# jaesung-cs/vulkan_radix_sort

Measured on AMD Instinct MI355X. Metric: GItems/s at N=2^25 (keys & key+value); achieved HBM GB/s vs peak, higher is better.
Workload: dtype u32

## Files before the change

### vulkan_radix_sort_amd/csrc/vrdx_kernels.hip

```cpp
#include <hip/hip_runtime.h>
#include <stdint.h>

#include <type_traits>

#include "vrdx_kernels.h"
#include "vrdx_layout.h"

namespace vrdx {



#ifdef VRDX_TRACE
#define VRDX_STAMP(slot)                                      \
  do {                                                        \
    if (a.trace != nullptr && tid == 0) stamps[slot] = wall_clock64(); \
  } while (0)
#else
#define VRDX_STAMP(slot) \
  do {                   \
  } while (0)
#endif


typedef uint32_t u32x4 __attribute__((ext_vector_type(4)));
typedef uint32_t u32x2 __attribute__((ext_vector_type(2)));
typedef u32x4 u32x4_a4 __attribute__((aligned(4)));

__device__ __forceinline__ uint32_t LoadStatus(const uint32_t* p) {
  return __hip_atomic_load(p, __ATOMIC_RELAXED, __HIP_MEMORY_SCOPE_AGENT);
}
__device__ __forceinline__ void StoreStatus(uint32_t* p, uint32_t v) {
  __hip_atomic_store(p, v, __ATOMIC_RELAXED, __HIP_MEMORY_SCOPE_AGENT);
}

__device__ __forceinline__ void AddToBlock(uint32_t* p, uint32_t count) {
  (void)__hip_atomic_fetch_add(p, count | (1u << VRDX_BLOCK_COUNT_SHIFT), __ATOMIC_RELAXED, __HIP_MEMORY_SCOPE_AGENT);
}

__device__ __forceinline__ uint32_t ElementCount(uint32_t maxCount, const uint32_t* countPtr) {
  if (countPtr == nullptr) return maxCount;
  const uint32_t c = *countPtr;
  return c < maxCount ? c : maxCount;
}

__device__ __forceinline__ uint64_t MatchDigit(uint32_t digit) {
  uint64_t mask = ~0ull;
#pragma unroll
  for (int b = 0; b < 8; ++b) {
    const bool bit = (digit >> b) & 1u;
    const uint64_t ballot = __ballot(bit);
    mask &= bit ? ballot : ~ballot;
  }
  return mask;
}

__device__ __forceinline__ uint32_t LanesBelow(uint64_t mask) {
  return __builtin_amdgcn_mbcnt_hi((uint32_t)(mask >> 32),
                                   __builtin_amdgcn_mbcnt_lo((uint32_t)mask, 0u));
}

__device__ __forceinline__ void LdsBarrier() {
  __builtin_amdgcn_fence(__ATOMIC_RELEASE, "workgroup", "local");
  __builtin_amdgcn_s_barrier();
  __builtin_amdgcn_fence(__ATOMIC_ACQUIRE, "workgroup", "local");
}

template <int KPT, bool NT = false, bool DYN = false>
__device__ __forceinline__ void LoadStriped(const uint32_t* base, uint32_t first, uint32_t n, bool full,
                                            uint32_t pad, uint32_t (&out)[KPT], uint32_t slots = KPT) {
  const char* const bytes = reinterpret_cast<const char*>(base);
  const uint32_t offset = first * 4u;
  auto word = [&](int i) {
    const uint32_t* const p = reinterpret_cast<const uint32_t*>(bytes + ((uint64_t)offset + (uint64_t)(i * 256)));
    return NT ? __builtin_nontemporal_load(p) : *p;
  };
  if (full) {
#pragma unroll
    for (int i = 0; i < KPT; ++i) {
      if (DYN && i % 4 == 0 && (uint32_t)i >= slots) break;
      out[i] = word(i);
    }
  } else {
#pragma unroll
    for (int i = 0; i < KPT; ++i) {
      if (DYN && i % 4 == 0 && (uint32_t)i >= slots) break;
      out[i] = first + i * 64 < n ? word(i) : pad;
    }
  }
}

__device__ __forceinline__ bool StreamingLoads(bool keyValue, uint32_t n) {
  return keyValue && n > kStreamingLoadsAbove && n <= kStreamingLoadsUpTo;
}

template <int KPT, bool DYN = false>
__device__ __forceinline__ void LoadTile(const uint32_t* base, uint32_t first, uint32_t n, bool full, uint32_t pad,
                                         uint32_t (&out)[KPT], bool streaming, uint32_t slots = KPT) {
  if (streaming) {
    asm volatile("; non-temporal tile loads" ::: "memory");
    LoadStriped<KPT, true, DYN>(base, first, n, full, pad, out, slots);
    asm volatile("" ::: "memory");
  } else {
    LoadStriped<KPT, false, DYN>(base, first, n, full, pad, out, slots);
  }
}

template <int KPT, bool DYN = false>
__device__ __forceinline__ void StoreStriped(uint32_t* base, uint32_t first, uint32_t n, bool full,
                                             const uint32_t (&in)[KPT], uint32_t slots = KPT) {
  char* const bytes = reinterpret_cast<char*>(base);
  const uint32_t offset = first * 4u;
#pragma unroll
  for (int i = 0; i < KPT; ++i) {
    if (DYN && i % 4 == 0 && (uint32_t)i >= slots) break;
    if (full || first + i * 64 < n)
      *reinterpret_cast<uint32_t*>(bytes + ((uint64_t)offset + (uint64_t)(i * 256))) = in[i];
  }
}

struct PassPlan {
  bool skip;
  bool copy;
  bool fromScratch;
  uint32_t digit;
};


template <int THREADS>
struct PassCounts {
  uint32_t v[(VRDX_PASSES * VRDX_RADIX) / THREADS];
};

template <int THREADS>
__device__ __forceinline__ PassCounts<THREADS> LoadPassCounts(const uint32_t* histogramTable, int tid) {
  PassCounts<THREADS> c;
#pragma unroll
  for (int k = 0; k < (int)(VRDX_PASSES * VRDX_RADIX) / THREADS; ++k) c.v[k] = histogramTable[tid + k * THREADS];
  return c;
}

template <int THREADS>
__device__ __forceinline__ void PublishPassVotes(const PassCounts<THREADS>& c, uint32_t n, uint32_t hybridCap, int tid,
                                                 uint32_t* flags) {
#pragma unroll
  for (int k = 0; k < (int)(VRDX_PASSES * VRDX_RADIX) / THREADS; ++k) {
    const int group = (tid + k * THREADS) >> 6;
    const uint64_t any = __ballot(c.v[k] == n);
    const uint64_t over = __ballot(c.v[k] > hybridCap);
    if ((tid & 63) == 0) {
      flags[group] = any != 0ull ? 1u : 0u;
      flags[16 + group] = over != 0ull ? 1u : 0u;
    }
  }
}

__device__ __forceinline__ uint32_t TrivialPasses(const uint32_t* flags) {
  uint32_t trivial = 0;
#pragma unroll
  for (uint32_t q = 0; q < VRDX_PASSES; ++q)
    if ((flags[4 * q] | flags[4 * q + 1] | flags[4 * q + 2] | flags[4 * q + 3]) != 0) trivial |= 1u << q;
  return trivial;
}

__device__ __forceinline__ int HybridByte(const uint32_t* flags, uint32_t hybridCap) {
  if (hybridCap == 0) return -1;
  const uint32_t ranked = ~TrivialPasses(flags) & 15u;
  if (ranked == 0) return -1;
  const int top = 31 - __clz((int)ranked);
  const bool fits = (flags[16 + 4 * top] | flags[17 + 4 * top] | flags[18 + 4 * top] | flags[19 + 4 * top]) == 0;
  return fits ? top : -1;
}

__device__ __forceinline__ PassPlan ReadPassPlan(const uint32_t* flags, uint32_t pass, uint32_t hybridCap) {
  PassPlan plan;
  const int hybridByte = HybridByte(flags, hybridCap);
  if (hybridByte >= 0) {
    plan.skip = pass != 0;
    plan.copy = false;
    plan.fromScratch = false;
    plan.digit = (uint32_t)hybridByte;
    return plan;
  }
  const uint32_t trivial = TrivialPasses(flags);
  const uint32_t ranked = VRDX_PASSES - (uint32_t)__popc(trivial);
  const uint32_t copier = (ranked & 1u) ? (uint32_t)(__ffs(trivial) - 1) : VRDX_PASSES;
  const uint32_t changes = (~trivial & 15u) | (copier < VRDX_PASSES ? 1u << copier : 0u);
  plan.skip = ((changes >> pass) & 1u) == 0;
  plan.copy = !plan.skip && ((trivial >> pass) & 1u) != 0;
  plan.fromScratch = (__popc(changes & ((1u << pass) - 1u)) & 1) != 0;
  plan.digit = pass;
  return plan;
}

__device__ __forceinline__ uint32_t WaveInclusiveScan(uint32_t v) {
  int x = (int)v;
  x += __builtin_amdgcn_update_dpp(0, x, 0x111, 0xf, 0xf, true);
  x += __builtin_amdgcn_update_dpp(0, x, 0x112, 0xf, 0xf, true);
  x += __builtin_amdgcn_update_dpp(0, x, 0x114, 0xf, 0xf, true);
  x += __builtin_amdgcn_update_dpp(0, x, 0x118, 0xf, 0xf, true);
  x += __builtin_amdgcn_update_dpp(0, x, 0x142, 0xa, 0xf, false);
  x += __builtin_amdgcn_update_dpp(0, x, 0x143, 0xc, 0xf, false);
  return (uint32_t)x;
}

__device__ __forceinline__ uint32_t BlockExclusiveScan256(uint32_t v, uint32_t* scratch4, int tid) {
  const int lane = tid & 63;
  const int wave = tid >> 6;
  const uint32_t x = WaveInclusiveScan(v);
  if (wave < 4 && lane == 63) scratch4[wave] = x;
  LdsBarrier();
  uint32_t add = 0;
  if (wave < 4) {
#pragma unroll
    for (int w = 0; w < 3; ++w)
      if (w < wave) add += scratch4[w];
  }
  return x - v + add;
}

constexpr uint32_t kHistGroupVecs = kHistGroupKeys / 4;
static_assert(kHistGroupVecs == kHistThreads * 4, "four loads per lane and group");

template <bool NT>
__device__ __forceinline__ void HistFetch(const u32x4_a4* keys4, uint32_t group, uint32_t tid, uint32_t nvec,
                                          u32x4 (&k)[4]) {
#pragma unroll
  for (uint32_t u = 0; u < 4; ++u) {
    uint32_t i = group * kHistGroupVecs + u * kHistThreads + tid;
    i = i < nvec ? i : (nvec != 0 ? nvec - 1 : 0u);
    k[u] = NT ? __builtin_nontemporal_load(keys4 + i) : keys4[i];
  }
}

template <uint32_t COPIES>
__global__ __launch_bounds__(kHistThreads) void histogram_kernel(const uint32_t* __restrict__ keys,
                                                                  uint32_t maxCount,
                                                                  const uint32_t* countPtr,
                                                                  uint32_t* __restrict__ globalHistogram,
                                                                  uint32_t* __restrict__ tickets,
                                                                  u32x4* __restrict__ statusClear,
// ... 1768 lines not shown
        LdsBarrier();
      }
      auto finish = [&](uint32_t done) {
        if (done == nvec / tileVecs && tid < (n & 3u)) {
          const uint32_t one[1] = {keys[(nvec << 2) + tid]};
          count(formTag, kOne, one);
        }
        if constexpr (FORM != TABLES) {
          flush(done, window);
          window = window == top ? top + kTopHalf : top;
        }
      };
      if (two) {
        for (; tile < tiles; tile += step) {
          tally(formTag, tile, 0, a4, nvec);
          fetch(streaming, tile + step, 0, nvec, a4);
          tally(formTag, tile, 4, b4, nvec);
          fetch(streaming, tile + step, 4, nvec, b4);
          finish(tile);
        }
      } else {
        for (; tile < tiles; tile += 2 * step) {
          tally(formTag, tile, 0, a4, nvec);
          fetch(streaming, tile + 2 * step, 0, nvec, a4);
          finish(tile);
          tally(formTag, tile + step, 0, b4, nvec);
          fetch(streaming, tile + 3 * step, 0, nvec, b4);
          if (tile + step < tiles) finish(tile + step);
        }
      }
    };
    if (form == TOP)
      loop(std::integral_constant<uint32_t, TOP>{});
    else if (form == PREFIXED)
      loop(std::integral_constant<uint32_t, PREFIXED>{});
    else
      loop(std::integral_constant<uint32_t, TABLES>{});
  };
  if (n > kHistStreamingLoadsAbove) {
    asm volatile("; non-temporal key loads" ::: "memory");
    sweep(std::true_type{});
  } else {
    sweep(std::false_type{});
  }
  if (form == PREFIXED && likeRef != 0u) atomicAdd(&byte3[(ref >> 24) * C3 + (tid & (C3 - 1))], likeRef);
  __syncthreads();

  if (tid < 3 * VRDX_RADIX) {
    uint32_t sum = 0;
#pragma unroll
    for (uint32_t c = 0; c < COPIES; ++c) sum += bins[tid * COPIES + ((c + tid) & (COPIES - 1))];
    if (sum != 0) atomicAdd(&a.histogramTable[tid], sum);
  } else {
    const uint32_t v = tid - 3 * VRDX_RADIX;
    uint32_t sum = 0;
    if (form == TOP) {
#pragma unroll
      for (uint32_t q = 0; q < PER_BYTE; ++q) sum += bucketSize[v * PER_BYTE + q];
    } else if (form == PREFIXED) {
#pragma unroll
      for (uint32_t c = 0; c < C3; ++c) sum += byte3[v * C3 + ((c + tid) & (C3 - 1))];
    } else {
#pragma unroll
      for (uint32_t c = 0; c < COPIES; ++c) sum += top[v * COPIES + ((c + tid) & (COPIES - 1))];
    }
    if (sum != 0) atomicAdd(&a.histogramTable[tid], sum);
  }
  if (form == PREFIXED) {
    for (uint32_t d = tid; d < D; d += kHistThreads) {
      const uint32_t mine = bucketSize[d];
      if (mine != 0) atomicAdd(&a.bucketCount[d], mine);
    }
  }
  const uint32_t above = shift + BITS;
  const bool broken = form == PREFIXED ? (differs >> (above & 31u)) != 0u : (mode == kMsdModeIdentical && differs != 0u);
  if (__ballot(broken) != 0ull && lane == 0) atomicOr(a.overflowWord, kMsdDeclinePrefix);
}

template <uint32_t BITS>
__global__ __launch_bounds__(1024) void spine_msd_kernel(MsdArgs a) {
  constexpr uint32_t D = 1u << BITS, ROW = D / 2;
  constexpr uint32_t WORDS = 16, CHUNKS = 64, MAXROWS = kMsdMaxTiles / CHUNKS;
  __shared__ uint32_t sumLo[WORDS][CHUNKS], sumHi[WORDS][CHUNKS], total[2 * WORDS], below[16];
  const uint32_t tid = threadIdx.x;
  const uint32_t j = tid & (WORDS - 1), c = tid / WORDS;
  const uint32_t w = blockIdx.x * WORDS + j;
  const uint32_t rows = (a.tiles + CHUNKS - 1) / CHUNKS;
  const uint32_t r0 = c * rows;
  uint32_t* const column = a.tileCounts + w;
  const uint32_t decided = *a.overflowWord;

  {
    u32x4* const clear = reinterpret_cast<u32x4*>(a.statusClear);
    for (uint32_t i = blockIdx.x * 1024u + tid; i < a.statusVecs; i += gridDim.x * 1024u) clear[i] = u32x4{0u, 0u, 0u, 0u};
  }
  const uint32_t firstBucket = blockIdx.x * 2u * WORDS;
  uint32_t underTop = tid < 256u && tid < (firstBucket >> (BITS - 8u)) ? a.histogramTable[3u * VRDX_RADIX + tid] : 0u;
  uint32_t underSizes = 0;
#pragma unroll
  for (uint32_t d = tid; d < D; d += 1024u)
    if (d < firstBucket) underSizes += a.bucketCount[d];

  uint32_t v[MAXROWS];
#pragma unroll
  for (uint32_t k = 0; k < MAXROWS; ++k) v[k] = (k < rows && r0 + k < a.tiles) ? column[(size_t)(r0 + k) * ROW] : 0u;
  if ((decided & kMsdDeclineMask) != 0u || ((decided >> kMsdModeShift) & kMsdModeMask) != kMsdModePlan) return;
  const bool topWindow = ((decided >> kMsdShiftShift) & kMsdShiftMask) == 32u - BITS;
  uint32_t under = topWindow ? underTop : underSizes;
  uint32_t lo = 0, hi = 0;
#pragma unroll
  for (uint32_t k = 0; k < MAXROWS; ++k) {
    lo += v[k] & 0xFFFFu;
    hi += v[k] >> 16;
  }
  sumLo[j][c] = lo;
  sumHi[j][c] = hi;
  under = WaveInclusiveScan(under);
  if ((tid & 63u) == 63u) below[tid >> 6] = under;
  __syncthreads();
  {
    const uint32_t word = tid >> 6, chunk = tid & 63u;
    const uint32_t x = sumLo[word][chunk], y = sumHi[word][chunk];
    const uint32_t ix = WaveInclusiveScan(x), iy = WaveInclusiveScan(y);
    sumLo[word][chunk] = ix - x;
    sumHi[word][chunk] = iy - y;
    if (chunk == 63u) {
      total[2 * word] = ix;
      total[2 * word + 1] = iy;
    }
  }
  __syncthreads();
  lo = sumLo[j][c];
  hi = sumHi[j][c];
#pragma unroll
  for (uint32_t k = 0; k < MAXROWS; ++k) {
    if (k < rows && r0 + k < a.tiles) column[(size_t)(r0 + k) * ROW] = (lo & 0xFFFFu) | (hi << 16);
    lo += v[k] & 0xFFFFu;
    hi += v[k] >> 16;
  }
  if (tid < 64u) {
    const uint32_t mine = tid < 2 * WORDS ? total[tid] : 0u;
    const uint32_t inclusive = WaveInclusiveScan(mine);
    if (tid < 2 * WORDS) {
      uint32_t base = inclusive - mine;
#pragma unroll
      for (uint32_t q = 0; q < 16; ++q) base += below[q];
      a.bucketBase[firstBucket + tid] = base;
      if (topWindow) a.bucketCount[firstBucket + tid] = mine;
      if (mine > a.cap) atomicOr(a.overflowWord, kMsdDeclineBucket);
    }
  }
}

template <uint32_t BITS, bool KV>
__device__ __forceinline__ void ScatterMsdBody(const MsdArgs a) {
  constexpr int THREADS = 1024, KPT = 32, WAVES = THREADS / 64;
  constexpr uint32_t TILE = kMsdTileKeys, D = 1u << BITS, ROW = D / 2u;
  static_assert(THREADS * KPT == TILE && ROW <= (uint32_t)THREADS && WAVES * ROW <= TILE, "geometry");
  extern __shared__ __attribute__((aligned(16))) uint32_t smem[];
  uint32_t* const sorted = smem;
  uint32_t* const counters = smem;
  uint32_t* const tileOffset = smem + TILE;
  uint32_t* const scanScratch = tileOffset + D;

  const int tid = threadIdx.x;
  const int lane = tid & 63;
  const int wave = tid >> 6;
  const uint32_t n = ElementCount(a.maxCount, a.countPtr);
  const uint32_t perXcd = gridDim.x / 8u;
  const uint32_t tile = (blockIdx.x % 8u) * perXcd + blockIdx.x / 8u;
  const uint32_t slots = a.tileKeys / (uint32_t)THREADS;
  const uint32_t frame = a.tileKeys;
  const uint32_t tileStart = tile * frame;
  const uint32_t decided = *a.overflowWord;
  if ((decided & kMsdDeclineMask) != 0u) {
    if (blockIdx.x == 0 && tid == 0 && a.declinedPlans != nullptr) atomicAdd(a.declinedPlans, 1u);
    return;
  }
  const uint32_t SHIFT = (decided >> kMsdShiftShift) & kMsdShiftMask;
  if (((decided >> kMsdModeShift) & kMsdModeMask) == kMsdModeIdentical) {
    if (blockIdx.x == 0 && tid == 0) *a.planWord = kMsdVerdictSorted;
    return;
  }
  const uint32_t valid = tile < a.tiles && tileStart < n ? ((n - tileStart) < frame ? (n - tileStart) : frame) : 0u;
  const uint32_t tileEnd = tileStart + valid;
  const uint32_t loadBase = tileStart + wave * (slots * 64) + lane;
  uint32_t key[KPT];
  LoadStriped<KPT, true, true>(a.keysCaller, loadBase, tileEnd, valid == frame, 0xFFFFFFFFu, key, slots);
  uint32_t prefixWord = 0, base0 = 0, base1 = 0;
  if ((uint32_t)tid < ROW && valid != 0) {
    prefixWord = a.tileCounts[(size_t)tile * ROW + tid];
    base0 = a.bucketBase[2 * tid];
    base1 = a.bucketBase[2 * tid + 1];
  }
  if (blockIdx.x == 0 && tid == 0) *a.planWord = kMsdVerdictRuns | (SHIFT << kMsdShiftShift);
  if (valid == 0) return;

  uint32_t* const myRow = counters + wave * ROW;
#pragma unroll
  for (uint32_t i = 0; i < ROW / 256u; ++i) reinterpret_cast<u32x4*>(myRow)[lane + 64 * i] = u32x4{0u, 0u, 0u, 0u};
  uint32_t rank[KPT / 2];
  RankPacked16<KPT, true>(key, SHIFT, BITS, myRow, lane, rank, slots);
  ForgetDerivedValues<KPT>(key);
  LdsBarrier();

  uint32_t column[WAVES];
  const uint32_t totals = (uint32_t)tid < ROW ? ColumnRead<ROW, WAVES>(counters, tid, column) : 0u;
  const uint32_t count0 = totals & 0xFFFFu, count1 = totals >> 16;
  const uint32_t local0 = BlockExclusiveScanAll<THREADS>(count0 + count1, scanScratch, tid);
  const uint32_t local1 = local0 + count0;
  if ((uint32_t)tid < ROW) {
    ColumnBasesFrom<ROW, WAVES>(counters, tid, local0 | (local1 << 16), column);
    tileOffset[2 * tid] = base0 + (prefixWord & 0xFFFFu) - local0;
    tileOffset[2 * tid + 1] = base1 + (prefixWord >> 16) - local1;
  }
  LdsBarrier();
  PositionsPacked16<KPT, TILE, true>(key, SHIFT, BITS, myRow, rank, slots);
  LdsBarrier();
#pragma unroll
  for (int i = 0; i < KPT; ++i) {
    if (i % 4 == 0 && (uint32_t)i >= slots) break;
    sorted[(rank[i / 2] >> (16 * (i % 2))) & 0xFFFFu] = key[i];
  }
  LdsBarrier();
  uint32_t val[KV ? KPT : 1];
  if constexpr (KV)
    LoadStriped<KPT, true, true>(a.valuesCaller, loadBase, tileEnd, valid == frame, 0u, val, slots);

  constexpr int QUADS = KPT / 4;
  constexpr int B = 4;
  uint32_t quadDigits[KV ? QUADS : 1];
  uint32_t boundaryQuad[2] = {~0u, ~0u};
  uint32_t boundaryDigits[2][2] = {{0, 0}, {0, 0}};
  if ((uint32_t)tid < ROW) {
    if (count0 != 0 && (local0 & 3u) != 0 && local0 < valid) boundaryQuad[0] = local0 & ~3u;
    if (count1 != 0 && (local1 & 3u) != 0 && local1 < valid) boundaryQuad[1] = local1 & ~3u;
  }
  if (tid == 0 && (valid & 3u) != 0) boundaryQuad[0] = valid & ~3u;
  auto scatterQuads = [&](uint32_t* out, bool keysPhase) {
#pragma unroll
    for (int j0 = 0; j0 < QUADS; j0 += B) {
      if (4u * (uint32_t)j0 * THREADS >= valid) break;
      u32x4 w4[B];
      uint32_t o[B];
      bool whole[B];
#pragma unroll
      for (int b = 0; b < B; ++b) w4[b] = *reinterpret_cast<const u32x4*>(&sorted[4u * (tid + (j0 + b) * THREADS)]);
#pragma unroll
      for (int b = 0; b < B; ++b) {
        const int j = j0 + b;
        const uint32_t p = StagingSlot<TILE>(4u * (tid + j * THREADS));
        uint32_t d0, d3;
        if (keysPhase) {
          d0 = __builtin_amdgcn_ubfe(w4[b][0], SHIFT, BITS);
          d3 = __builtin_amdgcn_ubfe(w4[b][3], SHIFT, BITS);
          if constexpr (KV) quadDigits[j] = d0 | (d3 << 16);
        } else {
          d0 = quadDigits[KV ? j : 0] & 0xFFFFu;
          d3 = quadDigits[KV ? j : 0] >> 16;
        }
        whole[b] = p + 3 < valid && d0 == d3;
        o[b] = tileOffset[d0] + p;
        asm volatile("" : "+v"(o[b]));
      }
#pragma unroll
      for (int b = 0; b < B; ++b)
        if (whole[b]) StoreQuad(out, o[b], w4[b]);
    }
#pragma unroll
    for (int s = 0; s < 2; ++s) {
      if (boundaryQuad[s] == ~0u) continue;
      const u32x4 q = *reinterpret_cast<const u32x4*>(&sorted[StagingSlot<TILE>(boundaryQuad[s])]);
      if (keysPhase) {
        boundaryDigits[s][0] = __builtin_amdgcn_ubfe(q[0], SHIFT, BITS) | (__builtin_amdgcn_ubfe(q[1], SHIFT, BITS) << 16);
        boundaryDigits[s][1] = __builtin_amdgcn_ubfe(q[2], SHIFT, BITS) | (__builtin_amdgcn_ubfe(q[3], SHIFT, BITS) << 16);
      }
#pragma unroll
      for (int c = 0; c < 4; ++c) {
        const uint32_t d = (boundaryDigits[s][c / 2] >> (16 * (c % 2))) & 0xFFFFu;
        if (boundaryQuad[s] + c < valid) StoreWord(out, tileOffset[d] + boundaryQuad[s] + c, q[c]);
      }
    }
  };
  scatterQuads(a.keysScratch, true);
  if constexpr (KV) {
    LdsBarrier();
#pragma unroll
    for (int i = 0; i < KPT; ++i) {
      if (i % 4 == 0 && (uint32_t)i >= slots) break;
      sorted[(rank[i / 2] >> (16 * (i % 2))) & 0xFFFFu] = val[i];
    }
    LdsBarrier();
    scatterQuads(a.valuesScratch, false);
  }
}

template <uint32_t BITS>
__device__ __forceinline__ void ScatterMsdPairBody(const MsdArgs a) {
  constexpr int THREADS = 1024, KPT = 32, WAVES = THREADS / 64;
  constexpr uint32_t TILE = kMsdTileKeys, D = 1u << BITS, ROW = D / 2u;
  static_assert(2 * WAVES * ROW <= TILE, "both sub-tiles' counter rows inside the staging buffer");
  extern __shared__ __attribute__((aligned(16))) uint32_t smem[];
  uint32_t* const sorted = smem;
  uint32_t* const counters = smem;
  uint32_t* const tileOffset = smem + TILE;
  uint32_t* const scanScratch = tileOffset + D;

  const int tid = threadIdx.x;
  const int lane = tid & 63;
  const int wave = tid >> 6;
  const uint32_t n = ElementCount(a.maxCount, a.countPtr);
  const uint32_t pairs = (a.tiles + 1u) / 2u;
  const uint32_t perXcd = (pairs + 7u) / 8u;
  const uint32_t pair = (blockIdx.x % 8u) * perXcd + blockIdx.x / 8u;
  const uint32_t slots = a.tileKeys / (uint32_t)THREADS;
  const uint32_t frame = a.tileKeys;
  const uint32_t decided = *a.overflowWord;
  if ((decided & kMsdDeclineMask) != 0u) {
    if (blockIdx.x == 0 && tid == 0 && a.declinedPlans != nullptr) atomicAdd(a.declinedPlans, 1u);
    return;
  }
  const uint32_t SHIFT = (decided >> kMsdShiftShift) & kMsdShiftMask;
  if (((decided >> kMsdModeShift) & kMsdModeMask) == kMsdModeIdentical) {
    if (blockIdx.x == 0 && tid == 0) *a.planWord = kMsdVerdictSorted;
    return;
  }
  const uint32_t tileA = 2u * pair;
  const uint32_t startA = tileA * frame, startB = startA + frame;
  const bool exists = blockIdx.x < 8u * perXcd && pair < pairs && startA < n;
  const uint32_t left = exists ? n - startA : 0u;
  const uint32_t validA = left < frame ? left : frame;
  const uint32_t validB = left > frame ? (left - frame < frame ? left - frame : frame) : 0u;
  const uint32_t valid = validA + validB;
  const uint32_t baseA = startA + wave * (slots * 64) + lane, baseB = baseA + frame;
  uint32_t keyA[KPT], keyB[KPT];
  LoadStriped<KPT, true, true>(a.keysCaller, baseA, startA + validA, validA == frame, 0xFFFFFFFFu, keyA, slots);
  LoadStriped<KPT, true, true>(a.keysCaller, baseB, startB + validB, validB == frame, 0xFFFFFFFFu, keyB, slots);
  uint32_t prefixWord = 0, base0 = 0, base1 = 0;
  if ((uint32_t)tid < ROW && valid != 0) {
    prefixWord = a.tileCounts[(size_t)tileA * ROW + tid];
    base0 = a.bucketBase[2 * tid];
    base1 = a.bucketBase[2 * tid + 1];
  }
  if (blockIdx.x == 0 && tid == 0) *a.planWord = kMsdVerdictRuns | (SHIFT << kMsdShiftShift);
  if (valid == 0) return;

  uint32_t* const rowA = counters + wave * ROW;
  uint32_t* const rowB = counters + (WAVES + wave) * ROW;
#pragma unroll
  for (uint32_t i = 0; i < ROW / 256u; ++i) {
    reinterpret_cast<u32x4*>(rowA)[lane + 64 * i] = u32x4{0u, 0u, 0u, 0u};
    reinterpret_cast<u32x4*>(rowB)[lane + 64 * i] = u32x4{0u, 0u, 0u, 0u};
  }
  uint32_t posA[KPT / 2], posB[KPT / 2];
  RankPacked16<KPT, true>(keyA, SHIFT, BITS, rowA, lane, posA, slots);
  ForgetDerivedValues<KPT>(keyA);
  RankPacked16<KPT, true>(keyB, SHIFT, BITS, rowB, lane, posB, slots);
  ForgetDerivedValues<KPT>(keyB);
  LdsBarrier();

  const uint32_t totals = (uint32_t)tid < ROW ? ColumnTotals<ROW, 2 * WAVES>(counters, tid) : 0u;
  const uint32_t count0 = totals & 0xFFFFu, count1 = totals >> 16;
  const uint32_t local0 = BlockExclusiveScanAll<THREADS>(count0 + count1, scanScratch, tid);
  const uint32_t local1 = local0 + count0;
  if ((uint32_t)tid < ROW) {
    ColumnBases<ROW, 2 * WAVES>(counters, tid, local0 | (local1 << 16));
    tileOffset[2 * tid] = base0 + (prefixWord & 0xFFFFu) - local0;
    tileOffset[2 * tid + 1] = base1 + (prefixWord >> 16) - local1;
  }
  LdsBarrier();
  PositionsPacked16<KPT, TILE, true, true>(keyA, SHIFT, BITS, rowA, posA, slots);
  PositionsPacked16<KPT, TILE, true, true>(keyB, SHIFT, BITS, rowB, posB, slots);
  LdsBarrier();

  constexpr int QUADS = KPT / 4;
  constexpr int B = 2;
  uint32_t boundaryQuad[2] = {~0u, ~0u};
  if ((uint32_t)tid < ROW) {
    if (count0 != 0 && (local0 & 3u) != 0 && local0 < valid) boundaryQuad[0] = local0 & ~3u;
    if (count1 != 0 && (local1 & 3u) != 0 && local1 < valid) boundaryQuad[1] = local1 & ~3u;
  }
  if (tid == 0 && (valid & 3u) != 0) boundaryQuad[0] = valid & ~3u;
#pragma unroll 1
  for (uint32_t half = 0; half < 2; ++half) {
    const uint32_t from = half * frame;
    if (from >= valid) break;
    if (half != 0) LdsBarrier();
#pragma unroll
    for (int i = 0; i < KPT; ++i) {
      if (i % 4 == 0 && (uint32_t)i >= slots) break;
      const uint32_t pa = ((posA[i / 2] >> (16 * (i % 2))) & 0xFFFFu) - from;
      const uint32_t pb = ((posB[i / 2] >> (16 * (i % 2))) & 0xFFFFu) - from;
      if (pa < frame) sorted[StagingSlot<TILE>(pa)] = keyA[i];
      if (pb < frame) sorted[StagingSlot<TILE>(pb)] = keyB[i];
    }
    LdsBarrier();
    const uint32_t here = valid - from < frame ? valid - from : frame;
#pragma unroll
    for (int j0 = 0; j0 < QUADS; j0 += B) {
      if (4u * (uint32_t)j0 * THREADS >= here) break;
      u32x4 w4[B];
      uint32_t o[B];
      bool whole[B];
#pragma unroll
      for (int b = 0; b < B; ++b) w4[b] = *reinterpret_cast<const u32x4*>(&sorted[4u * (tid + (j0 + b) * THREADS)]);
#pragma unroll
      for (int b = 0; b < B; ++b) {
        const uint32_t p = StagingSlot<TILE>(4u * (tid + (j0 + b) * THREADS));
        const uint32_t d0 = __builtin_amdgcn_ubfe(w4[b][0], SHIFT, BITS), d3 = __builtin_amdgcn_ubfe(w4[b][3], SHIFT, BITS);
        whole[b] = p + 3 < here && d0 == d3;
        o[b] = tileOffset[d0] + from + p;
        asm volatile("" : "+v"(o[b]));
      }
#pragma unroll
      for (int b = 0; b < B; ++b)
        if (whole[b]) StoreQuad(a.keysScratch, o[b], w4[b]);
    }
#pragma unroll
    for (int s = 0; s < 2; ++s) {
      const uint32_t q0 = boundaryQuad[s] - from;
      if (boundaryQuad[s] == ~0u || q0 >= frame) continue;
      const u32x4 q = *reinterpret_cast<const u32x4*>(&sorted[StagingSlot<TILE>(q0)]);
#pragma unroll
      for (int c = 0; c < 4; ++c)
        if (q0 + c < here) StoreWord(a.keysScratch, tileOffset[__builtin_amdgcn_ubfe(q[c], SHIFT, BITS)] + boundaryQuad[s] + c, q[c]);
    }
  }
}
template <uint32_t BITS, bool KV>
constexpr bool MsdScatterTakesPairs() { return !KV && BITS == 10; }
template <uint32_t BITS, bool KV>
__device__ __forceinline__ void ScatterMsdRole(const MsdArgs a) {
  if constexpr (MsdScatterTakesPairs<BITS, KV>())
    ScatterMsdPairBody<BITS>(a);
  else
    ScatterMsdBody<BITS, KV>(a);
}


template <uint32_t BITS, int KPT, bool KV, int THREADS = 1024>
__device__ __forceinline__ void BucketSort2Bucket(const MsdArgs a, const uint32_t bucket, const uint32_t below, const bool streamOut) {
  constexpr int WAVES = THREADS / 64;
  static_assert(THREADS == 1024 || THREADS == 512, "one or two words of a counter row per thread");
  constexpr uint32_t TILE = THREADS * KPT;
  constexpr uint32_t ROW = 1024;
  static_assert(32u - BITS <= 22u, "two passes of at most eleven bits");
  static_assert(TILE <= 65536 && WAVES * ROW <= TILE && KPT % 4 == 0, "packed positions; the staging buffer covers the counters");
  extern __shared__ __attribute__((aligned(16))) uint32_t smem[];
  uint32_t* const staged = smem;
  uint32_t* const counters = smem;
  uint32_t* const scanScratch = smem + TILE;

  const int tid = threadIdx.x;
  const int lane = tid & 63;
  const int wave = tid >> 6;
  const uint32_t W0 = (below + 1u) / 2u, W1 = below / 2u;
  constexpr uint32_t passes = 2u;
  const uint32_t myBase = (uint32_t)__builtin_amdgcn_readfirstlane((int)a.bucketBase[bucket]);
  const uint32_t n = (uint32_t)__builtin_amdgcn_readfirstlane((int)a.bucketCount[bucket]);
  if (n == 0) return;
  const uint32_t* const keysIn = a.keysScratch + myBase;
  uint32_t* const keysOut = a.keysCaller + myBase;
  const uint32_t* const valuesIn = KV ? a.valuesScratch + myBase : nullptr;
  uint32_t* const valuesOut = KV ? a.valuesCaller + myBase : nullptr;

  constexpr bool DYN = true;
  const uint32_t chunks = (n + 255u) / 256u;
  const uint32_t base = chunks / WAVES, extra = chunks % WAVES;
  const uint32_t w = (uint32_t)__builtin_amdgcn_readfirstlane(wave);
  const uint32_t slots = 4u * (base + (w < extra ? 1u : 0u));
  const uint32_t first = 256u * (w * base + (w < extra ? w : extra)) + lane;
  uint32_t key[KPT];
  uint32_t val[KV ? KPT : 1];
  LoadStriped<KPT, false, DYN>(keysIn, first, n, false, 0xFFFFFFFFu, key, slots);
  if constexpr (KV) LoadStriped<KPT, false, DYN>(valuesIn, first, n, false, 0u, val, slots);

  uint32_t* const myRow = counters + wave * ROW;
#pragma unroll 1
  for (uint32_t pass = 0; pass < passes; ++pass) {
    const uint32_t shift = pass == 0 ? 0u : W0;
    const uint32_t width = pass == 0 ? W0 : W1;
    const uint32_t words = width > 1u ? 1u << (width - 1u) : 1u;
#pragma unroll
    for (uint32_t i = 0; i < ROW / 256u; ++i)
      if (256u * i < words) reinterpret_cast<u32x4*>(myRow)[lane + 64 * i] = u32x4{0u, 0u, 0u, 0u};
    uint32_t rank[KPT / 2];
    RankPacked16<KPT, DYN>(key, shift, width, myRow, lane, rank, slots);
    ForgetDerivedValues<KPT>(key);
    LdsBarrier();
    uint32_t firstNow = first;
    asm volatile("" : "+v"(firstNow));
    if constexpr (THREADS == 512) {
      const bool mine = KV || 2u * (uint32_t)tid < words;
      u32x2 column[WAVES];
      const u32x2 totals = mine ? ColumnPairRead<ROW, WAVES>(counters, tid, column) : u32x2{0u, 0u};
      const uint32_t count0 = totals[0] & 0xFFFFu, count1 = totals[0] >> 16, count2 = totals[1] & 0xFFFFu;
      const uint32_t local0 = BlockExclusiveScanAll<THREADS>(count0 + count1 + count2 + (totals[1] >> 16), scanScratch + 16 * pass, tid);
      const uint32_t local2 = local0 + count0 + count1;
      if (mine)
        ColumnPairBasesFrom<ROW, WAVES>(counters, tid, u32x2{local0 | ((local0 + count0) << 16), local2 | ((local2 + count2) << 16)}, column);
    } else if constexpr (!KV) {
      const bool mine = (uint32_t)tid < words;
      uint32_t column[WAVES];
      const uint32_t totals = mine ? ColumnRead<ROW, WAVES>(counters, tid, column) : 0u;
      const uint32_t count0 = totals & 0xFFFFu;
      const uint32_t local0 = BlockExclusiveScanAll<THREADS>(count0 + (totals >> 16), scanScratch + 16 * pass, tid);
      if (mine) ColumnBasesFrom<ROW, WAVES>(counters, tid, local0 | ((local0 + count0) << 16), column);
    } else {
      const bool mine = (uint32_t)tid < words;
      const uint32_t totals = mine ? ColumnTotals<ROW, WAVES>(counters, tid) : 0u;
      const uint32_t count0 = totals & 0xFFFFu;
      const uint32_t local0 = BlockExclusiveScanAll<THREADS>(count0 + (totals >> 16), scanScratch + 16 * pass, tid);
      if (mine) ColumnBases<ROW, WAVES>(counters, tid, local0 | ((local0 + count0) << 16));
    }
    LdsBarrier();
    PositionsPacked16<KPT, TILE, DYN>(key, shift, width, myRow, rank, slots);
    LdsBarrier();
#pragma unroll
    for (int i = 0; i < KPT; ++i) {
      if (DYN && i % 4 == 0 && (uint32_t)i >= slots) break;
      staged[(rank[i / 2] >> (16 * (i % 2))) & 0xFFFFu] = key[i];
    }
    LdsBarrier();
#pragma unroll
    for (int i = 0; i < KPT; ++i) {
      if (DYN && i % 4 == 0 && (uint32_t)i >= slots) break;
      key[i] = staged[StagingSlot<TILE>(firstNow + 64 * i)];
    }
    if constexpr (KV) {
      LdsBarrier();
#pragma unroll
      for (int i = 0; i < KPT; ++i) {
        if (DYN && i % 4 == 0 && (uint32_t)i >= slots) break;
        staged[(rank[i / 2] >> (16 * (i % 2))) & 0xFFFFu] = val[i];
      }
      LdsBarrier();
#pragma unroll
      for (int i = 0; i < KPT; ++i) {
        if (DYN && i % 4 == 0 && (uint32_t)i >= slots) break;
        val[i] = staged[StagingSlot<TILE>(firstNow + 64 * i)];
      }
    }
    LdsBarrier();
  }
  if (KV ? a.maxCount > kStreamingLoadsAbove : streamOut) {
    asm volatile("; non-temporal output" ::: "memory");
#pragma unroll
    for (int i = 0; i < KPT; ++i) {
      if (DYN && i % 4 == 0 && (uint32_t)i >= slots) break;
      const uint32_t index = first + 64 * i;
      if (index < n) {
        __builtin_nontemporal_store(key[i], &keysOut[index]);
        if constexpr (KV) __builtin_nontemporal_store(val[i], &valuesOut[index]);
      }
    }
    asm volatile("" ::: "memory");
  } else {
#pragma unroll
    for (int i = 0; i < KPT; ++i) {
      if (DYN && i % 4 == 0 && (uint32_t)i >= slots) break;
      const uint32_t index = first + 64 * i;
      if (index < n) {
        keysOut[index] = key[i];
        if constexpr (KV) valuesOut[index] = val[i];
      }
    }
  }
}

template <uint32_t BITS, int KPT, bool KV, int THREADS = 1024>
__device__ __forceinline__ void BucketSort2Body(const MsdArgs a, const uint32_t workgroups) {
  const uint32_t verdict = *a.planWord;
  if ((verdict & kMsdVerdictMask) != kMsdVerdictRuns) return;
  const uint32_t below = (verdict >> kMsdShiftShift) & kMsdShiftMask;
  uint32_t streamedBuckets = 0u;
  if constexpr (!KV && THREADS == 1024 && BITS == 10)
    if (a.maxCount > kStreamingLoadsAbove) streamedBuckets = (1u << BITS) - min(a.plainTail, 1u << BITS);
#pragma unroll 1
  for (uint32_t bucket = blockIdx.x; bucket < (1u << BITS); bucket += workgroups)
    BucketSort2Bucket<BITS, KPT, KV, THREADS>(a, bucket, below, bucket < streamedBuckets);
}

template <uint32_t BITS, bool KV>
__global__ __launch_bounds__(512, 4) void bucket_sort2_half_kernel(MsdArgs a) {
  BucketSort2Body<BITS, kMsdHalfCap / 512, KV, 512>(a, gridDim.x);
}

template <uint32_t BITS, bool KV, bool DYN>
__device__ __forceinline__ void FallbackPassBody(const OnesweepArgs p) {
  if constexpr (KV)
    OnesweepBody<1024, 32, true, true, DYN>(p);
  else
    OnesweepPairBody<1024, 32, DYN>(p);
}

template <uint32_t BITS, bool KV, bool DYN>
__global__ __launch_bounds__(1024) void msd_scatter_or_pass0_kernel(MsdArgs m, OnesweepArgs p) {
  if ((*m.overflowWord & kMsdDeclineMask) == 0u) {
    ScatterMsdRole<BITS, KV>(m);
    return;
  }
  if (blockIdx.x > p.statusRows) return;
  FallbackPassBody<BITS, KV, DYN>(p);
  if (blockIdx.x == 0 && threadIdx.x == 0 && m.declinedPlans != nullptr) atomicAdd(m.declinedPlans, 1u);
}
template <uint32_t BITS, bool KV, bool DYN>
__global__ __launch_bounds__(1024) void msd_buckets_or_pass1_kernel(MsdArgs m, OnesweepArgs p) {
  const uint32_t verdict = *m.planWord & kMsdVerdictMask;
  if (verdict < kMsdVerdictRuns) {
    if (blockIdx.x > p.statusRows) return;
    FallbackPassBody<BITS, KV, DYN>(p);
    return;
  }
  const uint32_t workgroups = min(gridDim.x, (1u << BITS) / 2u);
  if (verdict == kMsdVerdictRuns && blockIdx.x < workgroups)
    BucketSort2Body<BITS, (KV ? kMsdCapKeyValue : kMsdCapKeys) / 1024, KV>(m, workgroups);
}

__device__ __forceinline__ uint32_t OrderCheckKey(uint32_t tid, uint32_t wave, uint32_t slot) {
  uint32_t x = (blockIdx.x * 1024u + tid) * 0x9E3779B9u + slot * 0x85EBCA6Bu;
  x ^= x >> 15; x *= 0x2C1B3C6Du; x ^= x >> 12; x *= 0x297A2D39u; x ^= x >> 15;
  const uint32_t mode = (blockIdx.x + wave + slot) % 6u;
  const uint32_t mask = mode == 0 ? 0u : mode == 1 ? 1u : mode == 2 ? 3u : mode == 3 ? 15u : mode == 4 ? 0x21u : 255u;
  return x & mask;
}

__global__ __launch_bounds__(1024) void lds_order_check_kernel(uint32_t* mismatches, uint32_t* sticky) {
  __shared__ uint32_t counters[2 * 16 * 256];
// ... 825 lines not shown
```

Measured before the change: 148.1.

## Interleave key-value pairs in MSD scatter scratch and load pairs in bucket sort

For key+value sorts, the MSD scatter now stages keys and values together as 8-byte pairs in LDS, in two half-tile trips, and writes them interleaved into the key scratch buffer. The downstream bucket sort then reads each key and value with one 8-byte load. The goal is to replace the separate keys and values scatter phases and their two scattered streams with one wider, better-coalesced stream. The cost is an extra LDS round and barrier per tile and a scratch buffer that must hold twice as many words. Any other consumer of valuesScratch is not visible here and may be inconsistent with the new layout.

```diff
diff --git a/vulkan_radix_sort_amd/csrc/vrdx_kernels.hip b/vulkan_radix_sort_amd/csrc/vrdx_kernels.hip
--- a/vulkan_radix_sort_amd/csrc/vrdx_kernels.hip
+++ b/vulkan_radix_sort_amd/csrc/vrdx_kernels.hip
@@ -86,6 +86,22 @@
       if (DYN && i % 4 == 0 && (uint32_t)i >= slots) break;
       out[i] = first + i * 64 < n ? word(i) : pad;
     }
+  }
+}
+
+template <int KPT, bool DYN = false>
+__device__ __forceinline__ void LoadStripedPairs(const uint32_t* pairs, uint32_t first, uint32_t n, uint32_t padKey,
+                                                 uint32_t padValue, uint32_t (&key)[KPT], uint32_t (&val)[KPT],
+                                                 uint32_t slots = KPT) {
+  const char* const bytes = reinterpret_cast<const char*>(pairs);
+  const uint32_t offset = first * 8u;
+#pragma unroll
+  for (int i = 0; i < KPT; ++i) {
+    if (DYN && i % 4 == 0 && (uint32_t)i >= slots) break;
+    u32x2 pair = {padKey, padValue};
+    if (first + i * 64 < n) pair = *reinterpret_cast<const u32x2*>(bytes + ((uint64_t)offset + (uint64_t)(i * 512)));
+    key[i] = pair[0];
+    val[i] = pair[1];
   }
 }
 
@@ -2160,7 +2176,7 @@
   }
 }
 
-template <uint32_t BITS, bool KV>
+template <uint32_t BITS>
 __device__ __forceinline__ void ScatterMsdBody(const MsdArgs a) {
   constexpr int THREADS = 1024, KPT = 32, WAVES = THREADS / 64;
   constexpr uint32_t TILE = kMsdTileKeys, D = 1u << BITS, ROW = D / 2u;
@@ -2231,13 +2247,9 @@
     sorted[(rank[i / 2] >> (16 * (i % 2))) & 0xFFFFu] = key[i];
   }
   LdsBarrier();
-  uint32_t val[KV ? KPT : 1];
-  if constexpr (KV)
-    LoadStriped<KPT, true, true>(a.valuesCaller, loadBase, tileEnd, valid == frame, 0u, val, slots);
 
   constexpr int QUADS = KPT / 4;
   constexpr int B = 4;
-  uint32_t quadDigits[KV ? QUADS : 1];
   uint32_t boundaryQuad[2] = {~0u, ~0u};
   uint32_t boundaryDigits[2][2] = {{0, 0}, {0, 0}};
   if ((uint32_t)tid < ROW) {
@@ -2245,7 +2257,7 @@
     if (count1 != 0 && (local1 & 3u) != 0 && local1 < valid) boundaryQuad[1] = local1 & ~3u;
   }
   if (tid == 0 && (valid & 3u) != 0) boundaryQuad[0] = valid & ~3u;
-  auto scatterQuads = [&](uint32_t* out, bool keysPhase) {
+  auto scatterQuads = [&](uint32_t* out) {
 #pragma unroll
     for (int j0 = 0; j0 < QUADS; j0 += B) {
       if (4u * (uint32_t)j0 * THREADS >= valid) break;
@@ -2258,15 +2270,7 @@
       for (int b = 0; b < B; ++b) {
         const int j = j0 + b;
         const uint32_t p = StagingSlot<TILE>(4u * (tid + j * THREADS));
-        uint32_t d0, d3;
-        if (keysPhase) {
-          d0 = __builtin_amdgcn_ubfe(w4[b][0], SHIFT, BITS);
-          d3 = __builtin_amdgcn_ubfe(w4[b][3], SHIFT, BITS);
-          if constexpr (KV) quadDigits[j] = d0 | (d3 << 16);
-        } else {
-          d0 = quadDigits[KV ? j : 0] & 0xFFFFu;
-          d3 = quadDigits[KV ? j : 0] >> 16;
-        }
+        const uint32_t d0 = __builtin_amdgcn_ubfe(w4[b][0], SHIFT, BITS), d3 = __builtin_amdgcn_ubfe(w4[b][3], SHIFT, BITS);
         whole[b] = p + 3 < valid && d0 == d3;
         o[b] = tileOffset[d0] + p;
         asm volatile("" : "+v"(o[b]));
@@ -2279,10 +2283,8 @@
     for (int s = 0; s < 2; ++s) {
       if (boundaryQuad[s] == ~0u) continue;
       const u32x4 q = *reinterpret_cast<const u32x4*>(&sorted[StagingSlot<TILE>(boundaryQuad[s])]);
-      if (keysPhase) {
-        boundaryDigits[s][0] = __builtin_amdgcn_ubfe(q[0], SHIFT, BITS) | (__builtin_amdgcn_ubfe(q[1], SHIFT, BITS) << 16);
-        boundaryDigits[s][1] = __builtin_amdgcn_ubfe(q[2], SHIFT, BITS) | (__builtin_amdgcn_ubfe(q[3], SHIFT, BITS) << 16);
-      }
+      boundaryDigits[s][0] = __builtin_amdgcn_ubfe(q[0], SHIFT, BITS) | (__builtin_amdgcn_ubfe(q[1], SHIFT, BITS) << 16);
+      boundaryDigits[s][1] = __builtin_amdgcn_ubfe(q[2], SHIFT, BITS) | (__builtin_amdgcn_ubfe(q[3], SHIFT, BITS) << 16);
 #pragma unroll
       for (int c = 0; c < 4; ++c) {
         const uint32_t d = (boundaryDigits[s][c / 2] >> (16 * (c % 2))) & 0xFFFFu;
@@ -2290,19 +2292,132 @@
       }
     }
   };
-  scatterQuads(a.keysScratch, true);
-  if constexpr (KV) {
+  scatterQuads(a.keysScratch);
+}
+
+__device__ __forceinline__ uint32_t PairStagingSlot(uint32_t p) { return p ^ ((p >> 4) & 0x1Eu); }
+__device__ __forceinline__ void StorePair(uint32_t* pairs, uint32_t index, u32x2 pair) {
+  *reinterpret_cast<u32x2*>(reinterpret_cast<char*>(pairs) + (uint64_t)(index * 8u)) = pair;
+}
+__device__ __forceinline__ void StorePairQuad(uint32_t* pairs, uint32_t index, u32x4 quad) {
+  *reinterpret_cast<u32x4_a4*>(reinterpret_cast<char*>(pairs) + (uint64_t)(index * 8u)) = quad;
+}
+template <uint32_t BITS>
+__device__ __forceinline__ void ScatterMsdKvBody(const MsdArgs a) {
+  constexpr int THREADS = 1024, KPT = 32, WAVES = THREADS / 64;
+  constexpr uint32_t TILE = kMsdTileKeys, D = 1u << BITS, ROW = D / 2u, H = TILE / 2u;
+  static_assert(THREADS * KPT == TILE && ROW <= (uint32_t)THREADS && WAVES * ROW <= TILE, "geometry");
+  extern __shared__ __attribute__((aligned(16))) uint32_t smem[];
+  uint32_t* const counters = smem;
+  uint32_t* const tileOffset = smem + TILE;
+  uint32_t* const scanScratch = tileOffset + D;
+
+  const int tid = threadIdx.x;
+  const int lane = tid & 63;
+  const int wave = tid >> 6;
+  const uint32_t n = ElementCount(a.maxCount, a.countPtr);
+  const uint32_t perXcd = gridDim.x / 8u;
+  const uint32_t tile = (blockIdx.x % 8u) * perXcd + blockIdx.x / 8u;
+  const uint32_t slots = a.tileKeys / (uint32_t)THREADS;
+  const uint32_t frame = a.tileKeys;
+  const uint32_t tileStart = tile * frame;
+  const uint32_t decided = *a.overflowWord;
+  if ((decided & kMsdDeclineMask) != 0u) {
+    if (blockIdx.x == 0 && tid == 0 && a.declinedPlans != nullptr) atomicAdd(a.declinedPlans, 1u);
+    return;
+  }
+  const uint32_t SHIFT = (decided >> kMsdShiftShift) & kMsdShiftMask;
+  if (((decided >> kMsdModeShift) & kMsdModeMask) == kMsdModeIdentical) {
+    if (blockIdx.x == 0 && tid == 0) *a.planWord = kMsdVerdictSorted;
+    return;
+  }
+  const uint32_t valid = tile < a.tiles && tileStart < n ? ((n - tileStart) < frame ? (n - tileStart) : frame) : 0u;
+  const uint32_t tileEnd = tileStart + valid;
+  const uint32_t loadBase = tileStart + wave * (slots * 64) + lane;
+  uint32_t key[KPT];
+  LoadStriped<KPT, true, true>(a.keysCaller, loadBase, tileEnd, valid == frame, 0xFFFFFFFFu, key, slots);
+  uint32_t prefixWord = 0, base0 = 0, base1 = 0;
+  if ((uint32_t)tid < ROW && valid != 0) {
+    prefixWord = a.tileCounts[(size_t)tile * ROW + tid];
+    base0 = a.bucketBase[2 * tid];
+    base1 = a.bucketBase[2 * tid + 1];
+  }
+  if (blockIdx.x == 0 && tid == 0) *a.planWord = kMsdVerdictRuns | (SHIFT << kMsdShiftShift);
+  if (valid == 0) return;
+
+  uint32_t* const myRow = counters + wave * ROW;
+#pragma unroll
+  for (uint32_t i = 0; i < ROW / 256u; ++i) reinterpret_cast<u32x4*>(myRow)[lane + 64 * i] = u32x4{0u, 0u, 0u, 0u};
+  uint32_t position[KPT / 2];
+  RankPacked16<KPT, true>(key, SHIFT, BITS, myRow, lane, position, slots);
+  ForgetDerivedValues<KPT>(key);
+  uint32_t val[KPT];
+  LoadStriped<KPT, true, true>(a.valuesCaller, loadBase, tileEnd, valid == frame, 0u, val, slots);
+  LdsBarrier();
+
+  const uint32_t totals = (uint32_t)tid < ROW ? ColumnTotals<ROW, WAVES>(counters, tid) : 0u;
+  const uint32_t count0 = totals & 0xFFFFu;
+  const uint32_t local0 = BlockExclusiveScanAll<THREADS>(count0 + (totals >> 16), scanScratch, tid);
+  const uint32_t local1 = local0 + count0;
+  if ((uint32_t)tid < ROW) {
+    ColumnBases<ROW, WAVES>(counters, tid, local0 | (local1 << 16));
+    tileOffset[2 * tid] = base0 + (prefixWord & 0xFFFFu) - local0;
+    tileOffset[2 * tid + 1] = base1 + (prefixWord >> 16) - local1;
+  }
+  LdsBarrier();
+  PositionsPacked16<KPT, TILE, true, true>(key, SHIFT, BITS, myRow, position, slots);
+  LdsBarrier();
+
+  constexpr int QUADS = (int)(H / 2u) / THREADS;
+  constexpr int B = 4;
+#pragma unroll 1
+  for (uint32_t trip = 0; trip < 2; ++trip) {
+    const uint32_t from = trip * H;
+    if (from >= valid) break;
+    if (trip != 0) LdsBarrier();
+    ForgetDerivedValues<KPT / 2>(position);
+    uint32_t me = (uint32_t)tid;
+    asm volatile("" : "+v"(me));
+    StaticFor<0, KPT, 4>([&](auto chunk) {
+      constexpr int base = decltype(chunk)::value;
+      if ((uint32_t)base >= slots) return false;
+#pragma unroll
+      for (int c = 0; c < 4; ++c) {
+        const int i = base + c;
+        const uint32_t p = ((position[i / 2] >> (16 * (i % 2))) & 0xFFFFu) - from;
+        if (p < H) reinterpret_cast<u32x2*>(smem)[PairStagingSlot(p)] = u32x2{key[i], val[i]};
+      }
+      return true;
+    });
     LdsBarrier();
-#pragma unroll
-    for (int i = 0; i < KPT; ++i) {
-      if (i % 4 == 0 && (uint32_t)i >= slots) break;
-      sorted[(rank[i / 2] >> (16 * (i % 2))) & 0xFFFFu] = val[i];
-    }
-    LdsBarrier();
-    scatterQuads(a.valuesScratch, false);
-  }
-}
-
+    const uint32_t here = valid - from < H ? valid - from : H;
+#pragma unroll
+    for (int j0 = 0; j0 < QUADS; j0 += B) {
+      if (2u * (uint32_t)j0 * THREADS >= here) break;
+      u32x4 w4[B];
+      uint32_t o0[B], o1[B];
+#pragma unroll
+      for (int b = 0; b < B; ++b) w4[b] = *reinterpret_cast<const u32x4*>(&smem[4u * (me + (j0 + b) * THREADS)]);
+#pragma unroll
+      for (int b = 0; b < B; ++b) {
+        o0[b] = tileOffset[__builtin_amdgcn_ubfe(w4[b][0], SHIFT, BITS)];
+        o1[b] = tileOffset[__builtin_amdgcn_ubfe(w4[b][2], SHIFT, BITS)];
+        asm volatile("" : "+v"(o0[b]), "+v"(o1[b]));
+      }
+#pragma unroll
+      for (int b = 0; b < B; ++b) {
+        const uint32_t p = PairStagingSlot(2u * (me + (j0 + b) * THREADS));
+        const uint32_t at = from + p;
+        if (p + 1 < here && o0[b] == o1[b]) {
+          StorePairQuad(a.keysScratch, o0[b] + at, w4[b]);
+        } else {
+          if (p < here) StorePair(a.keysScratch, o0[b] + at, u32x2{w4[b][0], w4[b][1]});
+          if (p + 1 < here) StorePair(a.keysScratch, o1[b] + at + 1u, u32x2{w4[b][2], w4[b][3]});
+        }
+      }
+    }
+  }
+}
 template <uint32_t BITS>
 __device__ __forceinline__ void ScatterMsdPairBody(const MsdArgs a) {
   constexpr int THREADS = 1024, KPT = 32, WAVES = THREADS / 64;
@@ -2439,10 +2554,12 @@
 constexpr bool MsdScatterTakesPairs() { return !KV && BITS == 10; }
 template <uint32_t BITS, bool KV>
 __device__ __forceinline__ void ScatterMsdRole(const MsdArgs a) {
-  if constexpr (MsdScatterTakesPairs<BITS, KV>())
+  if constexpr (KV)
+    ScatterMsdKvBody<BITS>(a);
+  else if constexpr (MsdScatterTakesPairs<BITS, KV>())
     ScatterMsdPairBody<BITS>(a);
   else
-    ScatterMsdBody<BITS, KV>(a);
+    ScatterMsdBody<BITS>(a);
 }
 
 
@@ -2467,9 +2584,8 @@
   const uint32_t myBase = (uint32_t)__builtin_amdgcn_readfirstlane((int)a.bucketBase[bucket]);
   const uint32_t n = (uint32_t)__builtin_amdgcn_readfirstlane((int)a.bucketCount[bucket]);
   if (n == 0) return;
-  const uint32_t* const keysIn = a.keysScratch + myBase;
+  const uint32_t* const keysIn = a.keysScratch + (KV ? 2u * (size_t)myBase : (size_t)myBase);
   uint32_t* const keysOut = a.keysCaller + myBase;
-  const uint32_t* const valuesIn = KV ? a.valuesScratch + myBase : nullptr;
   uint32_t* const valuesOut = KV ? a.valuesCaller + myBase : nullptr;
 
   constexpr bool DYN = true;
@@ -2480,8 +2596,10 @@
   const uint32_t first = 256u * (w * base + (w < extra ? w : extra)) + lane;
   uint32_t key[KPT];
   uint32_t val[KV ? KPT : 1];
-  LoadStriped<KPT, false, DYN>(keysIn, first, n, false, 0xFFFFFFFFu, key, slots);
-  if constexpr (KV) LoadStriped<KPT, false, DYN>(valuesIn, first, n, false, 0u, val, slots);
+  if constexpr (KV)
+    LoadStripedPairs<KPT, DYN>(keysIn, first, n, 0xFFFFFFFFu, 0u, key, val, slots);
+  else
+    LoadStriped<KPT, false, DYN>(keysIn, first, n, false, 0xFFFFFFFFu, key, slots);
 
   uint32_t* const myRow = counters + wave * ROW;
 #pragma unroll 1
```

Result: no change. 148.6, median of 3 (+0.3%).
